# hrpan/tetris_mcts

Hardware: AMD Instinct MI355X
Metric: mcts_node_expansions_per_sec (higher is better)
Workload: dtype f32

## Files before the change

### include/tetris_mcts_hip.h

```cpp
#ifndef TETRIS_MCTS_HIP_H
#define TETRIS_MCTS_HIP_H
#include <stdint.h>
#ifdef __cplusplus
extern "C" {
#endif

#define TM_NACT 7
#define TM_GAME_DW 16
#define TM_OBS_DW 12
#define TM_REC_DW 32
#define TM_REC_PCHILD 28
#define TM_REC_OBS 29
#define TM_REC_SCORE 30
#define TM_REC_HDR 31
#define TM_KIDS_DW 8
#define TM_GS_DW 64
#define TM_LEAF_DW 32
#define TM_DIST_ROW 64
#define TM_GC_PART_DW 192
#define TM_VALUENET_PARAMS 478342
#define TM_VALUENET_SCRATCH 9728
#define TM_VALUENET_SCRATCH_MFMA 2064
#define TM_VALUENET_PREPARED 477184
#define TM_VALUENET_PREPARED_X3 27648
#define TM_VALUENET_FP32 0
#define TM_VALUENET_BF16X3 1
#define TM_DISTNET_PARAMS(atoms) (279232 + 129 * (atoms))
#define TM_DISTNET_PARAMS_50 285682
#define TM_DISTNET_PREPARED 278528
#define TM_DISTNET_PREPARED_X3 24576
#define TM_DISTNET_SCRATCH 2048

enum {
    TM_GS_ROOT = 0, TM_GS_EPISODE, TM_GS_NFREE_NODE, TM_GS_NFREE_OBS, TM_GS_TRACE_LEN, TM_GS_PENDING,
    TM_GS_ERR, TM_GS_N_EXPAND, TM_GS_N_SIMS, TM_GS_N_GC, TM_GS_RNG_POS, TM_GS_N_NQ_FALLBACK,
    TM_GS_LEAF, TM_GS_LEAF_END, TM_GS_K_EVAL, TM_GS_LEAF_SCORE,
    TM_GS_TRACE_SUM,
    TM_GS_N_EVAL,
    TM_GS_N_POOL_RESET,
    TM_GS_MAX_TRACE,
    TM_GS_CYC_BACK = 20, TM_GS_CYC_SELECT, TM_GS_CYC_EXPAND,
    TM_GS_CYC_TAIL,
    TM_GS_N_DROPPED = 25,
    TM_GS_LOW_NODE = 26, TM_GS_LOW_OBS,
    TM_GS_FIRST_MISS = 28,
    TM_GS_PREFIX_SUM,
    TM_GS_GC_PHASE = 32,
    TM_GS_GC_ARRIVE,
    TM_GS_GC_ACTIVE4,
    TM_GS_GC_RSV1,
    TM_GS_GC_WORK,
    TM_GS_GC_MARK_LAUNCHES,
    TM_GS_GC_SLICES,
    TM_GS_GC_RETRY,
    TM_GS_SIM_TARGET = 40, TM_GS_SIM_STARTED,
    TM_GS_CYC_VERIFY,
    TM_GS_N_WALK_MISS,
    TM_GS_POOL_FULL,
    TM_GS_GC_IN_MOVE,
    TM_GS_GC_REQ_AT,
    TM_GS_LEAF_OBS,
    TM_GS_N_EVAL_SKIP,
    TM_GS_N_EVAL_CACHED,
    TM_GS_GC_NGC,
    TM_GS_GC_BLOCKS,
    TM_GS_GC_ITERS,
    TM_GS_GC_MARK_CYC,
    TM_GS_GC_FLAGS
    , TM_GS_GC_MARK_PARTS = 58,
    TM_GS_GC_MARK_SHARED,
    TM_GS_GC_CYC_LOAD,
    TM_GS_GC_CYC_ROUNDS,
    TM_GS_GC_CYC_WAVES,
    TM_GS_GC_IDLE_TURNS
};
#define TM_GC_FLAG_WORDS 4
#define TM_ERR_POOL 1
#define TM_ERR_TRACE 2
#define TM_ERR_TABLE 4
#define TM_ERR_EVAL_LIST 8
#define TM_ERR_GC_GRID 16

#define TM_KIND_VALUESIM 0
#define TM_KIND_VALUESIM_LP 1
#define TM_KIND_CPPAGENT_LP 2
#define TM_KIND_CPPAGENT 3
#define TM_KIND_VANILLA 4
#define TM_KIND_VANILLA_C 5
#define TM_KIND_DIST 6

typedef struct tm_store {
    int32_t n_games;
    int32_t max_nodes;
    int32_t table_cap;
    int32_t max_trace;
    int32_t eval_slots;
    int32_t nq_size;
    int32_t app, scoring, randomizer;
    int32_t low;
    int32_t kind;
    int32_t min_visits_to_store;
    int32_t online;
    int32_t replay_cap;
    int32_t gc_slice_cycles;
    double gamma;
    uint32_t *node_rec;
    uint32_t *node_game;
    uint32_t *obs_stat;
    uint32_t *obs_key;
    uint64_t *node_tab;
    uint64_t *obs_tab;
    int32_t *free_node;
    int32_t *free_obs;
    int32_t *gs;
    uint32_t *rng;
    uint32_t *env_game;
    int32_t *env_line_stats;
    uint32_t *trace;
    int32_t *leaf;
    int32_t *eval_obs;
    float *eval_v;
    float *eval_var;
    const float *nq_table;
    uint8_t *gc_mark;
    int32_t *gc_queue;
    uint32_t *replay_obs;
    float *replay_stat;
    int32_t *replay_count;
    uint32_t *mt_state;
    uint32_t *node_child;
    int32_t *gc_part;
    float *node_dist;
    float *eval_dist;
    const double *nq_table_d;
    double dist_vmin, dist_vmax;
    int32_t dist_bins;
    int32_t gc_spec_nodes;
    int32_t *eval_list;
    int32_t *eval_cnt;
    float *obs_eval;
    int32_t eval_parity;
    int32_t eval_epoch;
    float *replay_dist;
    const int32_t *game_list;
    int32_t n_listed;
    int32_t gc_cost_units;
    int32_t gc_collectors;
} tm_store;
#define TM_EVAL_SEGS(n_games) ((n_games) < 64 ? (n_games) : 64)

int tm_pool_init(const tm_store *s, void *stream);
int tm_pool_reset(const tm_store *s, const uint8_t *mask, void *stream);
void tm_fill_norm_quantile(float *host_table, int n);
void tm_fill_norm_quantile_f64(double *host_table, int n);

int tm_env_init(const tm_store *s, const uint32_t *seeds, void *stream);
int tm_env_step(const tm_store *s, const int32_t *actions, void *stream);
int tm_env_reset(const tm_store *s, const uint8_t *mask, void *stream);
int tm_env_render(const tm_store *s, int8_t *out , void *stream);
int tm_env_info(const tm_store *s, int32_t *out , void *stream);

int tm_update_root(const tm_store *s, void *stream);
int tm_tree_new_node(const tm_store *s, const uint32_t *games, const uint8_t *mask, int32_t *out_idx, void *stream);
int tm_tree_expand(const tm_store *s, const uint32_t *games, const uint8_t *mask, int32_t *out_idx, void *stream);
int tm_tree_remove_nodes(const tm_store *s, const uint8_t *mask, void *stream);
int tm_move_begin(const tm_store *s, int sims, void *stream);
int tm_sims_remaining(const tm_store *s, int32_t *out , void *stream);
int tm_sims_owing(const tm_store *s, int32_t *out , int32_t *list, void *stream);
int tm_gc_step(const tm_store *s, void *stream);
#define TM_SIM_BACKUP 1
#define TM_SIM_FRONT 2
#define TM_SIM_GC_FULL 4
#define TM_SIM_EVAL_NEEDED 8
#define TM_SIM_GC_MEM_MARKS 16
int tm_sim_step(const tm_store *s, int flags, void *stream);
int tm_eval_render(const tm_store *s, int8_t *out , void *stream);

int tm_store_slice(const tm_store *s, int first, int n, tm_store *out);

typedef struct tm_search tm_search;
int tm_search_create(tm_search **out, const tm_store *s, int n_sub, int ev_every);
void tm_search_destroy(tm_search *h);
int tm_search_run(tm_search *h, int sims, const float *vn_params, const float *vn_prepared, float *vn_scratch,
                  void *stream);
int tm_search_stats(tm_search *h, double *out, int n, int reset);
int tm_search_set_epoch(tm_search *h, int epoch);
int tm_search_set_valuenet(tm_search *h, int backend);
int tm_root_stats(const tm_store *s, float *stats , int32_t *action , void *stream);
int tm_export_game(const tm_store *s, int game, int32_t *child , float *score, int32_t *n_to_o,
                   int32_t *visit, float *value, float *variance, uint8_t *end_obs, void *stream);

int tm_core_select_trace_obs(int n_trees, int n_nodes, const int32_t *roots, const int32_t *child,
                             const int32_t *visit, const float *value, const float *variance, const float *score,
                             const int32_t *n_to_o, int low, uint32_t *rng, const float *nq_table, int nq_size,
                             int32_t *trace , int32_t *trace_len, int max_trace, void *stream);
int tm_core_backup_trace_obs(int n_trees, int n_nodes, const int32_t *trace, const int32_t *trace_len, int max_trace,
                             int32_t *visit, float *value, float *variance, const int32_t *n_to_o, const float *score,
                             const double *_value, const double *_variance, double gamma, void *stream);
int tm_core_backup_trace_obs_lp(int n_trees, int n_nodes, const int32_t *trace, const int32_t *trace_len,
                                int max_trace, int32_t *visit, float *value, float *variance, const int32_t *n_to_o,
                                const float *score, const uint8_t *end, const int32_t *_child ,
                                const int32_t *_obs, const int32_t *k, const float *_value, const float *_variance,
                                double gamma, int mixture, int averaged, void *stream);
int tm_core_get_unique_child_obs(int n_trees, int n_nodes, const int32_t *index, const int32_t *child,
                                 const float *score, const int32_t *n_to_o, int32_t *c_nodes ,
                                 int32_t *c_obs, int32_t *count, void *stream);
int tm_core_get_all_childs(int n_trees, int n_nodes, const int32_t *roots, const int32_t *child,
                           uint8_t *mark , int32_t *queue , void *stream);

int tm_dist_transform(int n, int bins, const float *dist , double vmin, double vmax,
                      const double *shift , double scale, float *out , void *stream);
int tm_dist_mean_variance(int n, int bins, const float *dist, double vmin, double vmax, double *out ,
                          void *stream);

int tm_distpy_shift(int n, int bins, const float *dist , const double *x , double vmin, double vmax,
                    float *out , void *stream);
int tm_distpy_policy(int n_trees, int n_nodes, const int32_t *child_nodes, const int32_t *n_child, const float *node_stats,
                     const double *curr_reward , int32_t *out , void *stream);
int tm_distpy_backup(int n_trees, int n_nodes, int bins, const int32_t *trace, const int32_t *trace_len, int max_trace,
                     float *node_stats, float *node_dist, const double *r , const float *leaf_dist ,
                     double vmin, double vmax, float *scratch, void *stream);

int tm_yogi_step(float *p, const float *g, float *m, float *v, double *state, int n, double lr, double beta1, double beta2,
                 double eps, double weight_decay, void *stream);
int tm_valuenet_prepare(const float *params, float *prepared, void *stream);
int tm_valuenet_forward(const float *params, const float *prepared, const int8_t *states, int n, float *v, float *var,
                        float *scratch, void *stream);
int tm_valuenet_forward_requests(const float *params, const float *prepared, const tm_store *s, float *scratch,
                                 void *stream);
int tm_valuenet_forward_plain(const float *params, const int8_t *states, int n, float *v, float *var, float *scratch,
                              void *stream);
int tm_valuenet_prepare_x3(const float *params, float *prepared_x3, void *stream);
int tm_valuenet_forward_x3(const float *params, const float *prepared, const float *prepared_x3, const int8_t *states, int n,
                           float *v, float *var, float *scratch, void *stream);
int tm_valuenet_forward_requests_x3(const float *params, const float *prepared, const float *prepared_x3, const tm_store *s,
                                    float *scratch, void *stream);

int tm_distnet_prepare(const float *params, float *prepared, void *stream);
int tm_distnet_forward(const float *params, const float *prepared, const int8_t *states, int n, int atoms, float *dist,
                       int dist_stride, float *scratch, void *stream);
int tm_distnet_forward_requests(const float *params, const float *prepared, const tm_store *s, float *scratch, void *stream);
int tm_distnet_prepare_x3(const float *params, float *prepared_x3, void *stream);
int tm_distnet_forward_x3(const float *params, const float *prepared, const float *prepared_x3, const int8_t *states,
                          int n, int atoms, float *dist, int dist_stride, float *scratch, void *stream);
int tm_distnet_forward_requests_x3(const float *params, const float *prepared, const float *prepared_x3,
                                   const tm_store *s, float *scratch, void *stream);

const char *tm_version(void);
int tm_store_layout(int *out, int n);
#ifdef __cplusplus
}
#endif
#endif
```

### tetris_mcts_amd/csrc/valuenet.hip

```cpp
#include <hip/hip_runtime.h>
#include <stdint.h>
#include <stdlib.h>
#include <mutex>
#include "../../include/tetris_mcts_hip.h"

namespace tmcts_vn {

constexpr int A1 = 32 * 18 * 8, A2 = 32 * 16 * 6, A3 = 32 * 14 * 4, HID = 256;
constexpr int OFF_C1W = 0, OFF_C1B = 288, OFF_C2W = 320, OFF_C2B = 9536, OFF_C3W = 9568, OFF_C3B = 18784,
              OFF_F1W = 18816, OFF_F1B = 477568, OFF_FOW = 477824, OFF_FOB = 478336, OFF_UB = 478338, OFF_LB = 478340;

__device__ inline double tm_exp(double x) {
    if (x > 700.0) x = 700.0;
    if (x < -700.0) x = -700.0;
    const double inv_ln2 = 1.4426950408889634074, ln2_hi = 6.93147180369123816490e-01,
                 ln2_lo = 1.90821492927058770002e-10;
    double n = rint(x * inv_ln2);
    double r = fma(-n, ln2_hi, x);
    r = fma(-n, ln2_lo, r);
    double p = 1.0 / 6227020800.0;
    p = fma(p, r, 1.0 / 479001600.0);
    p = fma(p, r, 1.0 / 39916800.0);
    p = fma(p, r, 1.0 / 3628800.0);
    p = fma(p, r, 1.0 / 362880.0);
    p = fma(p, r, 1.0 / 40320.0);
    p = fma(p, r, 1.0 / 5040.0);
    p = fma(p, r, 1.0 / 720.0);
    p = fma(p, r, 1.0 / 120.0);
    p = fma(p, r, 1.0 / 24.0);
    p = fma(p, r, 1.0 / 6.0);
    p = fma(p, r, 0.5);
    p = fma(p, r, 1.0);
    p = fma(p, r, 1.0);
    long long bits = __double_as_longlong(p);
    bits += ((long long)n) << 52;
    return __longlong_as_double(bits);
}

template <int CIN, int H, int W>
__global__ void k_conv3x3_relu(const float* __restrict__ in, int in_stride, const int8_t* __restrict__ in8,
                               const float* __restrict__ wt, const float* __restrict__ bias, float* __restrict__ out,
                               int out_stride, int n) {
    constexpr int OH = H - 2, OW = W - 2, PER = 32 * OH * OW;
    int t = blockIdx.x * blockDim.x + threadIdx.x;
    if (t >= n * PER) return;
    int s = t / PER, e = t - s * PER;
    int co = e / (OH * OW), p = e - co * (OH * OW), y = p / OW, x = p - y * OW;
    float acc = bias[co];
    for (int ci = 0; ci < CIN; ++ci)
        for (int ky = 0; ky < 3; ++ky)
            for (int kx = 0; kx < 3; ++kx) {
                int ii = (ci * H + y + ky) * W + x + kx;
                float xv = in8 ? (float)in8[(size_t)s * 200 + ii] : in[(size_t)s * in_stride + ii];
                acc = fmaf(xv, wt[((co * CIN + ci) * 3 + ky) * 3 + kx], acc);
            }
    out[(size_t)s * out_stride + e] = acc > 0.0f ? acc : 0.0f;
}

__global__ void k_fc1_relu(const float* __restrict__ a3, int stride, const float* __restrict__ w,
                           const float* __restrict__ b, float* __restrict__ h, int hstride, int n) {
    int t = blockIdx.x * blockDim.x + threadIdx.x;
    if (t >= n * HID) return;
    int s = t / HID, j = t - s * HID;
    float acc = b[j];
    const float* x = a3 + (size_t)s * stride;
    const float* wr = w + (size_t)j * A3;
    for (int i = 0; i < A3; ++i) acc = fmaf(x[i], wr[i], acc);
    h[(size_t)s * hstride + j] = acc > 0.0f ? acc : 0.0f;
}

__global__ void k_fc_out(const float* __restrict__ h, int hstride, const float* __restrict__ P, float* __restrict__ v,
                         float* __restrict__ var, int n, const int32_t* __restrict__ eval_obs) {
    int t = blockIdx.x * blockDim.x + threadIdx.x;
    if (t >= n * 2) return;
    int s = t >> 1, j = t & 1;
    if (eval_obs && eval_obs[s] == 0) return;
    float acc = P[OFF_FOB + j];
    const float* x = h + (size_t)s * hstride;
    const float* wr = P + OFF_FOW + j * HID;
    for (int i = 0; i < HID; ++i) acc = fmaf(x[i], wr[i], acc);
    double e = tm_exp(-(double)acc);
    float sg = (float)(1.0 / (1.0 + e));
    float tt = sg * P[OFF_UB + j];
    float o = tt + P[OFF_LB + j];
    if (j == 0) v[s] = o; else var[s] = o;
}

}
namespace tmcts_vn {

typedef float f32x16 __attribute__((ext_vector_type(16)));
constexpr int SCHED_REGION_QUADS = 6;
constexpr int PREP_W2 = 0, PREP_W3 = 9216, PREP_W1 = 18432, PREP_TOTAL = 18432 + 458752;
constexpr int A1CS = 145;
constexpr int A2CS = 97;
constexpr int CONV_WG_PER_CU = 2;
constexpr int WAVE_LDS = 32 * A1CS + 200;

__global__ void k_vn_prepare(const float* __restrict__ P, float* __restrict__ prep) {
    int t = blockIdx.x * blockDim.x + threadIdx.x;
    if (t < 2 * 9216) {
        const float* W = P + (t < 9216 ? OFF_C2W : OFF_C3W);
        int e = t % 9216;
        int q = e / 256, l = (e / 4) % 64, r = e % 4;
        int s = 4 * q + r;
        int k = 2 * s + (l >> 5), row = l & 31;
        prep[t] = W[row * 288 + k];
    } else if (t < PREP_TOTAL) {
        int e = t - 18432;
        int ht = e / (112 * 256), e2 = e % (112 * 256);
        int q = e2 / 256, l = (e2 / 4) % 64, r = e2 % 4;
        int s = 4 * q + r;
        int k = 4 * s + (l >> 4), row = 16 * ht + (l & 15);
        prep[t] = P[OFF_F1W + (size_t)row * A3 + k];
    }
}

__device__ __forceinline__ void lds_fence() {
    __builtin_amdgcn_fence(__ATOMIC_RELEASE, "wavefront");
    __builtin_amdgcn_wave_barrier();
    __builtin_amdgcn_fence(__ATOMIC_ACQUIRE, "wavefront");
}

template <int TILES, int IN_CS>
__device__ __forceinline__ void conv_mfma(const float* __restrict__ in, const int (&boff)[TILES][9],
                                          const float4* __restrict__ W, f32x16 (&acc)[TILES]) {
    float4 wq[3];
    float bb[2][4][TILES];
    auto load_b = [&](int q, int buf) {
#pragma unroll
        for (int r = 0; r < 4; ++r) {
            const int s = 4 * q + r, cp = s / 9, j = s % 9;
#pragma unroll
            for (int t = 0; t < TILES; ++t) bb[buf][r][t] = in[boff[t][j] + cp * 2 * IN_CS];
        }
    };
    wq[0] = W[0];
    wq[1] = W[64];
    load_b(0, 0);
#pragma unroll
    for (int q = 0; q < 36; ++q) {
        if (q + 2 < 36) wq[(q + 2) % 3] = W[(q + 2) * 64];
        if (q + 1 < 36) load_b(q + 1, (q + 1) & 1);
        const float4 w4 = wq[q % 3];
#pragma unroll
        for (int r = 0; r < 4; ++r) {
            const float a = (r == 0) ? w4.x : (r == 1) ? w4.y : (r == 2) ? w4.z : w4.w;
#pragma unroll
            for (int t = 0; t < TILES; ++t)
                acc[t] = __builtin_amdgcn_mfma_f32_32x32x2f32(a, bb[q & 1][r][t], acc[t], 0, 0, 0);
        }
        __builtin_amdgcn_sched_group_barrier(0x020, 1, 0);
#pragma unroll
        for (int i = 0; i < 4 * TILES; ++i) {
            __builtin_amdgcn_sched_group_barrier(0x008, 1, 0);
            __builtin_amdgcn_sched_group_barrier(0x100, 1, 0);
        }
        if (q % SCHED_REGION_QUADS == SCHED_REGION_QUADS - 1) __builtin_amdgcn_sched_barrier(0);
    }
}

constexpr int CONV_WAVES_PER_SIMD = 2;
struct ReqList {
    const int2* list;
    const int32_t* cnt;
    int parity, segs, slots;
};
__device__ __forceinline__ int req_prefix(const ReqList& rq, int lane, int& total) {
    int incl = lane < rq.segs ? rq.cnt[lane * 2 + rq.parity] : 0;
#pragma unroll
    for (int d = 1; d < 64; d <<= 1) {
        const int t = __shfl_up(incl, d, 64);
        if (lane >= d) incl += t;
    }
    total = __shfl(incl, 63, 64);
    return incl;
}
__device__ __forceinline__ int req_at(const ReqList& rq, int incl, int p, int lane) {
    const int sg = __popcll(__ballot(lane < rq.segs && incl <= p));
    const int before = __shfl(incl, sg > 0 ? sg - 1 : 0, 64);
    const int d = p - (sg > 0 ? before : 0);
    return (sg + rq.segs * (d / rq.slots)) * rq.slots + d % rq.slots;
}
__device__ __forceinline__ uint32_t req_obs_word(const ReqList& rq, int incl, const uint32_t* __restrict__ obs_key, int max_nodes,
                                                 int n, int p, int lane) {
    if (p >= n) return 0u;
    const int2 e = rq.list[req_at(rq, incl, p, lane)];
    return lane < 12 ? obs_key[((size_t)(e.x / rq.slots) * max_nodes + e.y) * 12 + lane] : 0u;
}
__device__ __forceinline__ void render_obs(uint32_t kw, int lane, float* x0) {
    const uint32_t cells = __shfl((int)kw, 10, 64), endw = __shfl((int)kw, 11, 64);
#pragma unroll
    for (int it = 0; it < 4; ++it) {
        const int i = lane + 64 * it, ic = min(i, 199);
        int r = ic / 10, c = ic - 10 * r;
        uint32_t w2 = (uint32_t)__shfl((int)kw, r >> 1, 64);
        float v = (float)((w2 >> (16 * (r & 1) + c)) & 1u);
        bool pc = ((cells & 0xFF) == (uint32_t)ic) | (((cells >> 8) & 0xFF) == (uint32_t)ic) |
                  (((cells >> 16) & 0xFF) == (uint32_t)ic) | ((cells >> 24) == (uint32_t)ic);
        if (!(endw & 0xFFu) && pc) v = -1.0f;
        if (i < 200) x0[i] = v;
    }
}
#include "valuenet_conv.inc"

typedef float f32x4 __attribute__((ext_vector_type(4)));
typedef float f32x4v __attribute__((ext_vector_type(4)));
#ifdef TM_FC1_TIMELINE
#define FC1_STAMP(i) do { if (threadIdx.x == 0 && s0 + (int)blockIdx.y < n) reinterpret_cast<int*>(hout)[(size_t)(s0 + blockIdx.y) * hstride + HID + 1 + (i)] = (int)__builtin_amdgcn_s_memrealtime(); } while (0)
#else
#define FC1_STAMP(i) do { } while (0)
#endif
template <int RT, int NY, int KC, int WRING, int PF>
__global__ __launch_bounds__(512) void k_vn_fc1(const float* __restrict__ P, const float* __restrict__ prep,
                                                const float* __restrict__ a3, int a3stride, int n,
                                                float* __restrict__ hout, int hstride,
                                                ReqList rq, int32_t* __restrict__ cnt, int cnt_stride,
                                                float* __restrict__ v_out, float* __restrict__ var_out) {
    constexpr int ROWS = 16 * RT, PITCH = KC + 4, HS_PITCH = HID + 4;
    constexpr int UNITS = HID / NY, HT = UNITS / 16, SG = 8 / HT, NST = RT / SG;
    static_assert(HT * SG == 8 && NST * SG == RT && NST >= 1 && ROWS <= 64, "eight waves = hidden tiles x groups of state tiles; one lane per row");
    constexpr int BT = ROWS * PITCH > (ROWS * HS_PITCH + 1) / 2 ? ROWS * PITCH : (ROWS * HS_PITCH + 1) / 2;
    __shared__ __attribute__((aligned(16))) float bt[2][BT];
    __shared__ int row_slot[ROWS];
    __shared__ int last_flag;
    const int w = threadIdx.x >> 6, lane = threadIdx.x & 63, kk = lane >> 4, l15 = lane & 15;
    const int s0 = blockIdx.x * ROWS;
    int my_slot = 0;
    FC1_STAMP(0);
    if (rq.list) {
        const int incl = req_prefix(rq, lane, n);
        if (s0 >= n) return;
        if (w == 0) {
            const int p = min(s0 + (lane & (ROWS - 1)), n - 1);
            int sg = 0;
            for (int k = 0; k < rq.segs; ++k) sg += __builtin_amdgcn_readlane(incl, k) <= p ? 1 : 0;
            const int before = __shfl(incl, sg > 0 ? sg - 1 : 0, 64);
            const int d = p - (sg > 0 ? before : 0);
            my_slot = rq.list[(sg + rq.segs * (d / rq.slots)) * rq.slots + d % rq.slots].x;
        }
    }
    const int ht = blockIdx.y * HT + (w % HT);
    const int st0 = (w / HT) * NST;
    const float4* W = reinterpret_cast<const float4*>(prep + PREP_W1) + (size_t)ht * 112 * 64 + lane;
    f32x4 acc[NST];
#pragma unroll
    for (int t = 0; t < NST; ++t)
#pragma unroll
        for (int r = 0; r < 4; ++r) acc[t][r] = P[OFF_F1B + 16 * ht + kk * 4 + r];
    constexpr int NCH = A3 / KC;
    constexpr int GRP = 16 / NST, QPG = GRP / 4, NGRP = KC / 4 / GRP;
    static_assert(A3 % KC == 0 && NCH >= 2 && (KC / 4) % GRP == 0, "chunking");
    float4 wring[WRING][QPG];
    auto wload = [&](int G) {
#pragma unroll
        for (int q = 0; q < QPG; ++q) wring[G % WRING][q] = W[((size_t)G * QPG + q) * 64];
    };
#pragma unroll
    for (int G0 = 0; G0 < WRING - 1; ++G0) wload(G0);
    constexpr int TPR = KC / 4, RPP = 512 / TPR, NPASS = ROWS / RPP;
    const int row0 = threadIdx.x / TPR, c4 = (threadIdx.x % TPR) * 4;
    float4 st[PF][NPASS];
    auto gload = [&](int chunk) {
#pragma unroll
        for (int i = 0; i < NPASS; ++i) {
            const int sa = s0 + row0 + RPP * i;
            st[chunk % PF][i] = (sa < n) ? *reinterpret_cast<const float4*>(a3 + (size_t)sa * a3stride + chunk * KC + c4)
                                         : make_float4(0, 0, 0, 0);
        }
    };
    auto lstore = [&](int chunk) {
#pragma unroll
        for (int i = 0; i < NPASS; ++i)
            *reinterpret_cast<float4*>(&bt[chunk & 1][(row0 + RPP * i) * PITCH + c4]) = st[chunk % PF][i];
    };
    static_assert(PF >= 2 && PF <= A3 / KC, "chunks in flight");
#pragma unroll
    for (int c = 0; c < PF; ++c) gload(c);
    FC1_STAMP(1);
    lstore(0);
    __syncthreads();
    FC1_STAMP(2);
#pragma unroll
    for (int c = 0; c < NCH; ++c) {
        if (c + PF < NCH) gload(c + PF);
        const float* b0 = &bt[c & 1][(16 * st0 + l15) * PITCH + kk];
        float bb[2][NST][GRP];
        auto load_b = [&](int grp, int buf) {
#pragma unroll
            for (int t = 0; t < NST; ++t)
#pragma unroll
                for (int i = 0; i < GRP; ++i) bb[buf][t][i] = b0[16 * t * PITCH + 4 * (GRP * grp + i)];
        };
        load_b(0, 0);
#pragma unroll
        for (int gq = 0; gq < NGRP; ++gq) {
            const int G = c * NGRP + gq;
            if (G + WRING - 1 < NCH * NGRP) wload(G + WRING - 1);
            if (gq + 1 < NGRP) load_b(gq + 1, (gq + 1) & 1);
#pragma unroll
            for (int i = 0; i < GRP; ++i) {
                const float4 w4 = wring[G % WRING][i / 4];
                const int r = i & 3;
                const float a = (r == 0) ? w4.x : (r == 1) ? w4.y : (r == 2) ? w4.z : w4.w;
#pragma unroll
                for (int t = 0; t < NST; ++t)
                    acc[t] = __builtin_amdgcn_mfma_f32_16x16x4f32(a, bb[gq & 1][t][i], acc[t], 0, 0, 0);
            }
#pragma unroll
            for (int i = 0; i < NST * GRP / 2; ++i) {
                __builtin_amdgcn_sched_group_barrier(0x008, 2, 0);
                __builtin_amdgcn_sched_group_barrier(0x100, 1, 0);
            }
            __builtin_amdgcn_sched_barrier(0);
        }
        if (c + 1 < NCH) lstore(c + 1);
        __syncthreads();
        if (c == NCH - 1) FC1_STAMP(3);
    }
    const int i0 = 16 * ht + kk * 4;
    float* hs = &bt[0][0];
    static_assert(ROWS * HS_PITCH <= 2 * BT, "hidden tile fits the staging buffers");
#pragma unroll
    for (int t = 0; t < NST; ++t) {
        f32x4v o0;
#pragma unroll
        for (int r = 0; r < 4; ++r) o0[r] = acc[t][r] > 0.f ? acc[t][r] : 0.f;
        const int row = 16 * (st0 + t) + l15;
        if (s0 + row < n) {
            float* dst = hout + (size_t)(s0 + row) * hstride + i0;
            asm volatile("global_store_dwordx4 %0, %1, off sc1" :: "v"(dst), "v"(o0) : "memory");
        }
        *reinterpret_cast<f32x4v*>(&hs[row * HS_PITCH + i0]) = o0;
    }
    if (rq.list && w == 0 && lane < ROWS) row_slot[lane] = my_slot;
    asm volatile("s_waitcnt vmcnt(0)" ::: "memory");
    __syncthreads();
    FC1_STAMP(4);
    if (threadIdx.x == 0) {
        const int old = __hip_atomic_fetch_add(&cnt[(size_t)blockIdx.x * cnt_stride], 1, __ATOMIC_RELAXED, __HIP_MEMORY_SCOPE_AGENT);
        last_flag = old;
        if (old == NY - 1) __hip_atomic_store(&cnt[(size_t)blockIdx.x * cnt_stride], 0, __ATOMIC_RELAXED, __HIP_MEMORY_SCOPE_AGENT);
    }
    __syncthreads();
    FC1_STAMP(5);
    if (last_flag != NY - 1) return;
    {
        constexpr int OQ = (HID - UNITS) / 4, CNT = ROWS * OQ / 512;
        static_assert(ROWS * OQ % 512 == 0, "whole passes");
        f32x4v wv[CNT];
#pragma unroll
        for (int i = 0; i < CNT; ++i) {
            const int e = i * 512 + threadIdx.x, row = e / OQ, c = (e % OQ) * 4;
            const int col = c < (int)blockIdx.y * UNITS ? c : c + UNITS;
            const float* src = hout + (size_t)(s0 + (s0 + row < n ? row : 0)) * hstride + col;
            asm volatile("global_load_dwordx4 %0, %1, off sc1" : "=v"(wv[i]) : "v"(src) : "memory");
        }
        asm volatile("s_waitcnt vmcnt(0)" ::: "memory");
#pragma unroll
        for (int i = 0; i < CNT; ++i) {
            const int e = i * 512 + threadIdx.x, row = e / OQ, c = (e % OQ) * 4;
            const int col = c < (int)blockIdx.y * UNITS ? c : c + UNITS;
            f32x4v t = wv[i];
            asm volatile("" : "+v"(t));
            if (s0 + row < n) *reinterpret_cast<f32x4v*>(&hs[row * HS_PITCH + col]) = t;
        }
    }
    __syncthreads();
    FC1_STAMP(6);
    if (threadIdx.x < 2 * ROWS) {
        const int j = threadIdx.x >> 1, o = threadIdx.x & 1;
        int sidx = s0 + j;
        const bool live = sidx < n;
        if (rq.list) sidx = row_slot[j];
        if (live) {
            float a = P[OFF_FOB + o];
            const float* x = &hs[j * HS_PITCH];
            const float* wr = P + OFF_FOW + o * HID;
            if ((reinterpret_cast<uintptr_t>(wr) & 15) == 0) {
                const float4* x4 = reinterpret_cast<const float4*>(x);
                const float4* w4 = reinterpret_cast<const float4*>(wr);
#pragma unroll 8
                for (int i = 0; i < HID / 4; ++i) {
                    const float4 xv = x4[i], wv = w4[i];
                    a = fmaf(xv.x, wv.x, a); a = fmaf(xv.y, wv.y, a); a = fmaf(xv.z, wv.z, a); a = fmaf(xv.w, wv.w, a);
                }
            } else {
#pragma unroll 8
                for (int i = 0; i < HID; ++i) a = fmaf(x[i], wr[i], a);
            }
            const double e = tm_exp(-(double)a);
            const float sg = (float)(1.0 / (1.0 + e));
            const float tt = sg * P[OFF_UB + o];
            const float res = tt + P[OFF_LB + o];
            if (o == 0) v_out[sidx] = res; else var_out[sidx] = res;
        }
    }
    FC1_STAMP(7);
}

#include "valuenet_x3.inc"

}

using namespace tmcts_vn;

extern "C" {

int tm_valuenet_prepare(const float* P, float* prepared, void* stream_) {
    hipLaunchKernelGGL(k_vn_prepare, dim3((PREP_TOTAL + 255) / 256), dim3(256), 0, (hipStream_t)stream_, P, prepared);
    return (int)hipGetLastError();
}

int tm_valuenet_forward_plain(const float* P, const int8_t* states, int n, float* v, float* var, float* scratch,
                              void* stream_) {
    hipStream_t stream = (hipStream_t)stream_;
    if (n <= 0) return 0;
    constexpr int SS = TM_VALUENET_SCRATCH;
    float* a1 = scratch;
    const int T = 256;
    hipLaunchKernelGGL((k_conv3x3_relu<1, 20, 10>), dim3((n * A1 + T - 1) / T), dim3(T), 0, stream, (const float*)nullptr,
                       0, states, P + OFF_C1W, P + OFF_C1B, a1, SS, n);
    hipLaunchKernelGGL((k_conv3x3_relu<32, 18, 8>), dim3((n * A2 + T - 1) / T), dim3(T), 0, stream, a1, SS,
                       (const int8_t*)nullptr, P + OFF_C2W, P + OFF_C2B, a1 + A1, SS, n);
    hipLaunchKernelGGL((k_conv3x3_relu<32, 16, 6>), dim3((n * A3 + T - 1) / T), dim3(T), 0, stream, a1 + A1, SS,
                       (const int8_t*)nullptr, P + OFF_C3W, P + OFF_C3B, a1 + A1 + A2, SS, n);
    hipLaunchKernelGGL(k_fc1_relu, dim3((n * HID + T - 1) / T), dim3(T), 0, stream, a1 + A1 + A2, SS, P + OFF_F1W,
                       P + OFF_F1B, a1 + A1 + A2 + A3, SS, n);
    hipLaunchKernelGGL(k_fc_out, dim3((n * 2 + T - 1) / T), dim3(T), 0, stream, a1 + A1 + A2 + A3, SS, P, v, var, n,
                       (const int32_t*)nullptr);
    return (int)hipGetLastError();
}

static int vn_forward_impl(const float* P, const float* prepared, const __bf16* planes, const int8_t* states,
                           const uint32_t* obs_key, const ReqList& rq, int max_nodes, int n, float* v, float* var,
                           float* scratch, hipStream_t stream) {
    if (n <= 0) return 0;
    constexpr int SS = TM_VALUENET_SCRATCH_MFMA;
    static_assert(SS >= A3 + HID + 1 && SS % 4 == 0, "scratch row");
    if (planes) {
        const int lds = 4 * X3_WAVE_BYTES;
        static std::once_flag x3_once;
        static int x3_err = 0;
        std::call_once(x3_once, [&] {
            x3_err = (int)hipFuncSetAttribute(reinterpret_cast<const void*>(k_vn_conv_x3),
                                              hipFuncAttributeMaxDynamicSharedMemorySize, lds);
        });
        if (x3_err) return x3_err;
        const int blocks = (n + 3) / 4 < 256 ? (n + 3) / 4 : 256;
        hipLaunchKernelGGL(k_vn_conv_x3, dim3(blocks), dim3(256), lds, stream, P, planes, states, obs_key, rq,
                           max_nodes, n, scratch, SS, reinterpret_cast<int32_t*>(scratch + A3 + HID), 32 * SS);
    } else {
        const int lds = 4 * WAVE_LDS * (int)sizeof(float);
        static std::once_flag attr_once;
        static int attr_err = 0;
        std::call_once(attr_once, [&] {
            attr_err = (int)hipFuncSetAttribute(reinterpret_cast<const void*>(k_vn_conv),
                                                hipFuncAttributeMaxDynamicSharedMemorySize, lds);
        });
        if (attr_err) return attr_err;
        int blocks = (n + 3) / 4;
        if (blocks > 256 * CONV_WG_PER_CU) blocks = 256 * CONV_WG_PER_CU;
        hipLaunchKernelGGL(k_vn_conv, dim3(blocks), dim3(256), lds, stream, P, prepared, states, obs_key, rq,
                           max_nodes, n, scratch, SS, reinterpret_cast<int32_t*>(scratch + A3 + HID), 32 * SS);
    }
    if (n >= 8192)
        hipLaunchKernelGGL((k_vn_fc1<4, 4, 128, 3, 2>), dim3((n + 63) / 64, 4), dim3(512), 0, stream, P, prepared, scratch, SS, n,
                           scratch + A3, SS, rq, reinterpret_cast<int32_t*>(scratch + A3 + HID), 64 * SS, v, var);
    else
        hipLaunchKernelGGL((k_vn_fc1<2, 4, 256, 6, 2>), dim3((n + 31) / 32, 4), dim3(512), 0, stream, P, prepared, scratch, SS, n,
                           scratch + A3, SS, rq, reinterpret_cast<int32_t*>(scratch + A3 + HID), 32 * SS, v, var);
    return (int)hipGetLastError();
}

int tm_valuenet_forward(const float* P, const float* prepared, const int8_t* states, int n, float* v, float* var,
                        float* scratch, void* stream_) {
    return vn_forward_impl(P, prepared, nullptr, states, nullptr, ReqList{nullptr, nullptr, 0, 0, 1}, 0, n, v, var, scratch,
                           (hipStream_t)stream_);
}

int tm_valuenet_forward_requests(const float* P, const float* prepared, const tm_store* s, float* scratch, void* stream_) {
    const ReqList rq{reinterpret_cast<const int2*>(s->eval_list), s->eval_cnt, s->eval_parity, TM_EVAL_SEGS(s->n_games), s->eval_slots};
    return vn_forward_impl(P, prepared, nullptr, nullptr, s->obs_key, rq, s->max_nodes,
                           s->n_games * s->eval_slots, s->eval_v, s->eval_var, scratch, (hipStream_t)stream_);
}

int tm_valuenet_prepare_x3(const float* P, float* prepared_x3, void* stream_) {
    if (!prepared_x3) return (int)hipErrorInvalidValue;
    hipLaunchKernelGGL(k_vn_prepare_x3, dim3((2 * 18 * 64 * 8 + 255) / 256), dim3(256), 0, (hipStream_t)stream_, P,
                       reinterpret_cast<__bf16*>(prepared_x3));
    return (int)hipGetLastError();
}

int tm_valuenet_forward_x3(const float* P, const float* prepared, const float* prepared_x3, const int8_t* states, int n, float* v,
                           float* var, float* scratch, void* stream_) {
    if (!prepared_x3) return (int)hipErrorInvalidValue;
    return vn_forward_impl(P, prepared, reinterpret_cast<const __bf16*>(prepared_x3), states, nullptr,
                           ReqList{nullptr, nullptr, 0, 0, 1}, 0, n, v, var, scratch, (hipStream_t)stream_);
}

int tm_valuenet_forward_requests_x3(const float* P, const float* prepared, const float* prepared_x3, const tm_store* s,
                                    float* scratch, void* stream_) {
    if (!prepared_x3) return (int)hipErrorInvalidValue;
    const ReqList rq{reinterpret_cast<const int2*>(s->eval_list), s->eval_cnt, s->eval_parity, TM_EVAL_SEGS(s->n_games), s->eval_slots};
    return vn_forward_impl(P, prepared, reinterpret_cast<const __bf16*>(prepared_x3), nullptr, s->obs_key, rq, s->max_nodes,
                           s->n_games * s->eval_slots, s->eval_v, s->eval_var, scratch, (hipStream_t)stream_);
}

}
```

Baseline: 20.32 million.

## Make valuenet fc1 a persistent grid dealing tile/part items across CUs

Replaces the 2D grid of fc1 blocks (tiles x hidden parts) with a persistent grid sized to resident workgroups per CU, where each block loops over (tile, part) items dealt in an XCD-aware order. The request prefix is computed once per block instead of per tile, and the output-layer weights are staged into LDS during the last chunk instead of read from global memory in the epilogue. Adds a waves-per-EU attribute and a non-inlined sigmoid to reduce register pressure. This targets launch overhead and tail imbalance, at the cost of extra per-item syncs and loop overhead.

```diff
diff --git a/include/tetris_mcts_hip.h b/include/tetris_mcts_hip.h
--- a/include/tetris_mcts_hip.h
+++ b/include/tetris_mcts_hip.h
@@ -230,6 +230,7 @@
                                  void *stream);
 int tm_valuenet_forward_plain(const float *params, const int8_t *states, int n, float *v, float *var, float *scratch,
                               void *stream);
+int tm_fc1_deal(int requests, int rows, int parts, int grid, int b, int32_t *items, int cap);
 int tm_valuenet_prepare_x3(const float *params, float *prepared_x3, void *stream);
 int tm_valuenet_forward_x3(const float *params, const float *prepared, const float *prepared_x3, const int8_t *states, int n,
                            float *v, float *var, float *scratch, void *stream);
diff --git a/tetris_mcts_amd/csrc/valuenet.hip b/tetris_mcts_amd/csrc/valuenet.hip
--- a/tetris_mcts_amd/csrc/valuenet.hip
+++ b/tetris_mcts_amd/csrc/valuenet.hip
@@ -206,13 +206,29 @@
 
 typedef float f32x4 __attribute__((ext_vector_type(4)));
 typedef float f32x4v __attribute__((ext_vector_type(4)));
+constexpr int FC1_XCDS = 8;
+struct Fc1Item { int tile, part; };
+__host__ __device__ constexpr int fc1_item_count(int requests, int rows, int parts) {
+    return requests > 0 ? (requests + rows - 1) / rows * parts : 0;
+}
+__host__ __device__ constexpr int fc1_item_index(int b, int grid, int k) { return b + k * grid; }
+__host__ __device__ constexpr Fc1Item fc1_item(int index, int requests, int rows, int parts) {
+    const int tiles = (requests + rows - 1) / rows, t8 = tiles / FC1_XCDS * FC1_XCDS, bulk = t8 * parts;
+    if (index < bulk) return Fc1Item{index % t8, index / t8};
+    const int rest = tiles - t8, j = index - bulk;
+    return Fc1Item{t8 + j % rest, j / rest};
+}
 #ifdef TM_FC1_TIMELINE
-#define FC1_STAMP(i) do { if (threadIdx.x == 0 && s0 + (int)blockIdx.y < n) reinterpret_cast<int*>(hout)[(size_t)(s0 + blockIdx.y) * hstride + HID + 1 + (i)] = (int)__builtin_amdgcn_s_memrealtime(); } while (0)
+#define FC1_STAMP(i) do { if (tid == 0 && s0 + part < n) reinterpret_cast<int*>(hout)[(size_t)(s0 + part) * hstride + HID + 1 + (i)] = (int)__builtin_amdgcn_s_memrealtime(); } while (0)
 #else
 #define FC1_STAMP(i) do { } while (0)
 #endif
+__device__ __noinline__ float fc1_sigmoid(float a) {
+    const double e = tm_exp(-(double)a);
+    return (float)(1.0 / (1.0 + e));
+}
 template <int RT, int NY, int KC, int WRING, int PF>
-__global__ __launch_bounds__(512) void k_vn_fc1(const float* __restrict__ P, const float* __restrict__ prep,
+__global__ __launch_bounds__(512) __attribute__((amdgpu_waves_per_eu(RT == 4 ? 4 : 2))) void k_vn_fc1(const float* __restrict__ P, const float* __restrict__ prep,
                                                 const float* __restrict__ a3, int a3stride, int n,
                                                 float* __restrict__ hout, int hstride,
                                                 ReqList rq, int32_t* __restrict__ cnt, int cnt_stride,
@@ -224,13 +240,25 @@
     __shared__ __attribute__((aligned(16))) float bt[2][BT];
     __shared__ int row_slot[ROWS];
     __shared__ int last_flag;
-    const int w = threadIdx.x >> 6, lane = threadIdx.x & 63, kk = lane >> 4, l15 = lane & 15;
-    const int s0 = blockIdx.x * ROWS;
+    constexpr int WO = 2 * HID + 6;
+    static_assert(OFF_FOB == OFF_FOW + 2 * HID && OFF_UB == OFF_FOB + 2 && OFF_LB == OFF_UB + 2, "the output layer's parameters are consecutive");
+    __shared__ __attribute__((aligned(16))) float wo[(WO + 3) / 4 * 4];
+    const int lane = threadIdx.x & 63;
+    int incl = 0;
+    if (rq.list) {
+        incl = req_prefix(rq, lane, n);
+        n = __builtin_amdgcn_readfirstlane(n);
+    }
+    const int n_items = fc1_item_count(n, ROWS, NY);
+    for (int item = fc1_item_index(blockIdx.x, gridDim.x, 0), kth = 0; item < n_items; item = fc1_item_index(blockIdx.x, gridDim.x, ++kth)) {
+    int tid = threadIdx.x;
+    asm volatile("" : "+v"(tid));
+    const int w = tid >> 6, lane = tid & 63, kk = lane >> 4, l15 = lane & 15;
+    const Fc1Item it = fc1_item(item, n, ROWS, NY);
+    const int tile = it.tile, part = it.part, s0 = tile * ROWS;
     int my_slot = 0;
     FC1_STAMP(0);
     if (rq.list) {
-        const int incl = req_prefix(rq, lane, n);
-        if (s0 >= n) return;
         if (w == 0) {
             const int p = min(s0 + (lane & (ROWS - 1)), n - 1);
             int sg = 0;
@@ -240,7 +268,7 @@
             my_slot = rq.list[(sg + rq.segs * (d / rq.slots)) * rq.slots + d % rq.slots].x;
         }
     }
-    const int ht = blockIdx.y * HT + (w % HT);
+    const int ht = part * HT + (w % HT);
     const int st0 = (w / HT) * NST;
     const float4* W = reinterpret_cast<const float4*>(prep + PREP_W1) + (size_t)ht * 112 * 64 + lane;
     f32x4 acc[NST];
@@ -259,7 +287,7 @@
 #pragma unroll
     for (int G0 = 0; G0 < WRING - 1; ++G0) wload(G0);
     constexpr int TPR = KC / 4, RPP = 512 / TPR, NPASS = ROWS / RPP;
-    const int row0 = threadIdx.x / TPR, c4 = (threadIdx.x % TPR) * 4;
+    const int row0 = tid / TPR, c4 = (tid % TPR) * 4;
     float4 st[PF][NPASS];
     auto gload = [&](int chunk) {
 #pragma unroll
@@ -275,6 +303,7 @@
             *reinterpret_cast<float4*>(&bt[chunk & 1][(row0 + RPP * i) * PITCH + c4]) = st[chunk % PF][i];
     };
     static_assert(PF >= 2 && PF <= A3 / KC, "chunks in flight");
+    float wo_r[4] = {0.f, 0.f, 0.f, 0.f};
 #pragma unroll
     for (int c = 0; c < PF; ++c) gload(c);
     FC1_STAMP(1);
@@ -284,6 +313,11 @@
 #pragma unroll
     for (int c = 0; c < NCH; ++c) {
         if (c + PF < NCH) gload(c + PF);
+        if (c == NCH - 1 && tid < (WO + 3) / 4) {
+#pragma unroll
+            for (int r = 0; r < 4; ++r)
+                if (4 * tid + r < WO) wo_r[r] = P[OFF_FOW + 4 * tid + r];
+        }
         const float* b0 = &bt[c & 1][(16 * st0 + l15) * PITCH + kk];
         float bb[2][NST][GRP];
         auto load_b = [&](int grp, int buf) {
@@ -334,33 +368,34 @@
         *reinterpret_cast<f32x4v*>(&hs[row * HS_PITCH + i0]) = o0;
     }
     if (rq.list && w == 0 && lane < ROWS) row_slot[lane] = my_slot;
+    if (tid < (WO + 3) / 4) *reinterpret_cast<float4*>(&wo[4 * tid]) = make_float4(wo_r[0], wo_r[1], wo_r[2], wo_r[3]);
     asm volatile("s_waitcnt vmcnt(0)" ::: "memory");
     __syncthreads();
     FC1_STAMP(4);
-    if (threadIdx.x == 0) {
-        const int old = __hip_atomic_fetch_add(&cnt[(size_t)blockIdx.x * cnt_stride], 1, __ATOMIC_RELAXED, __HIP_MEMORY_SCOPE_AGENT);
+    if (tid == 0) {
+        const int old = __hip_atomic_fetch_add(&cnt[(size_t)tile * cnt_stride], 1, __ATOMIC_RELAXED, __HIP_MEMORY_SCOPE_AGENT);
         last_flag = old;
-        if (old == NY - 1) __hip_atomic_store(&cnt[(size_t)blockIdx.x * cnt_stride], 0, __ATOMIC_RELAXED, __HIP_MEMORY_SCOPE_AGENT);
+        if (old == NY - 1) __hip_atomic_store(&cnt[(size_t)tile * cnt_stride], 0, __ATOMIC_RELAXED, __HIP_MEMORY_SCOPE_AGENT);
     }
     __syncthreads();
     FC1_STAMP(5);
-    if (last_flag != NY - 1) return;
+    if (last_flag == NY - 1) {
     {
         constexpr int OQ = (HID - UNITS) / 4, CNT = ROWS * OQ / 512;
         static_assert(ROWS * OQ % 512 == 0, "whole passes");
         f32x4v wv[CNT];
 #pragma unroll
         for (int i = 0; i < CNT; ++i) {
-            const int e = i * 512 + threadIdx.x, row = e / OQ, c = (e % OQ) * 4;
-            const int col = c < (int)blockIdx.y * UNITS ? c : c + UNITS;
+            const int e = i * 512 + tid, row = e / OQ, c = (e % OQ) * 4;
+            const int col = c < part * UNITS ? c : c + UNITS;
             const float* src = hout + (size_t)(s0 + (s0 + row < n ? row : 0)) * hstride + col;
             asm volatile("global_load_dwordx4 %0, %1, off sc1" : "=v"(wv[i]) : "v"(src) : "memory");
         }
         asm volatile("s_waitcnt vmcnt(0)" ::: "memory");
 #pragma unroll
         for (int i = 0; i < CNT; ++i) {
-            const int e = i * 512 + threadIdx.x, row = e / OQ, c = (e % OQ) * 4;
-            const int col = c < (int)blockIdx.y * UNITS ? c : c + UNITS;
+            const int e = i * 512 + tid, row = e / OQ, c = (e % OQ) * 4;
+            const int col = c < part * UNITS ? c : c + UNITS;
             f32x4v t = wv[i];
             asm volatile("" : "+v"(t));
             if (s0 + row < n) *reinterpret_cast<f32x4v*>(&hs[row * HS_PITCH + col]) = t;
@@ -368,35 +403,30 @@
     }
     __syncthreads();
     FC1_STAMP(6);
-    if (threadIdx.x < 2 * ROWS) {
-        const int j = threadIdx.x >> 1, o = threadIdx.x & 1;
+    if (tid < 2 * ROWS) {
+        const int j = tid >> 1, o = tid & 1;
         int sidx = s0 + j;
         const bool live = sidx < n;
         if (rq.list) sidx = row_slot[j];
         if (live) {
-            float a = P[OFF_FOB + o];
-            const float* x = &hs[j * HS_PITCH];
-            const float* wr = P + OFF_FOW + o * HID;
-            if ((reinterpret_cast<uintptr_t>(wr) & 15) == 0) {
-                const float4* x4 = reinterpret_cast<const float4*>(x);
-                const float4* w4 = reinterpret_cast<const float4*>(wr);
+            float a = wo[2 * HID + o];
+            const float4* x4 = reinterpret_cast<const float4*>(&hs[j * HS_PITCH]);
+            const float4* w4 = reinterpret_cast<const float4*>(&wo[o * HID]);
 #pragma unroll 8
-                for (int i = 0; i < HID / 4; ++i) {
-                    const float4 xv = x4[i], wv = w4[i];
-                    a = fmaf(xv.x, wv.x, a); a = fmaf(xv.y, wv.y, a); a = fmaf(xv.z, wv.z, a); a = fmaf(xv.w, wv.w, a);
-                }
-            } else {
-#pragma unroll 8
-                for (int i = 0; i < HID; ++i) a = fmaf(x[i], wr[i], a);
+            for (int i = 0; i < HID / 4; ++i) {
+                const float4 xv = x4[i], wv = w4[i];
+                a = fmaf(xv.x, wv.x, a); a = fmaf(xv.y, wv.y, a); a = fmaf(xv.z, wv.z, a); a = fmaf(xv.w, wv.w, a);
             }
-            const double e = tm_exp(-(double)a);
-            const float sg = (float)(1.0 / (1.0 + e));
-            const float tt = sg * P[OFF_UB + o];
-            const float res = tt + P[OFF_LB + o];
+            const float sg = fc1_sigmoid(a);
+            const float tt = sg * wo[2 * HID + 2 + o];
+            const float res = tt + wo[2 * HID + 4 + o];
             if (o == 0) v_out[sidx] = res; else var_out[sidx] = res;
         }
     }
     FC1_STAMP(7);
+    }
+    if (fc1_item_index(blockIdx.x, gridDim.x, kth + 1) < n_items) __syncthreads();
+    }
 }
 
 #include "valuenet_x3.inc"
@@ -404,6 +434,35 @@
 }
 
 using namespace tmcts_vn;
+
+static int vn_compute_units() {
+    static std::once_flag once;
+    static int cus = 0;
+    std::call_once(once, [&] {
+        int dev = 0;
+        if (hipGetDevice(&dev) != hipSuccess || hipDeviceGetAttribute(&cus, hipDeviceAttributeMultiprocessorCount, dev) != hipSuccess) cus = 0;
+    });
+    return cus;
+}
+
+template <int RT, int NY, int KC, int WRING, int PF, int WG_PER_CU>
+static int vn_fc1_launch_shape(const float* P, const float* prepared, const ReqList& rq, int n, float* v, float* var,
+                               float* scratch, hipStream_t stream) {
+    constexpr int SS = TM_VALUENET_SCRATCH_MFMA, ROWS = 16 * RT;
+    const int cus = vn_compute_units();
+    if (cus <= 0) return (int)hipErrorInvalidDevice;
+    const int items = fc1_item_count(n, ROWS, NY), resident = cus * WG_PER_CU;
+    hipLaunchKernelGGL((k_vn_fc1<RT, NY, KC, WRING, PF>), dim3(items < resident ? items : resident), dim3(512), 0, stream, P,
+                       prepared, scratch, SS, n, scratch + A3, SS, rq, reinterpret_cast<int32_t*>(scratch + A3 + HID), ROWS * SS,
+                       v, var);
+    return (int)hipGetLastError();
+}
+static int vn_fc1_launch(const float* P, const float* prepared, const ReqList& rq, int n, float* v, float* var, float* scratch,
+                         hipStream_t stream) {
+    if (n >= 8192)
+        return vn_fc1_launch_shape<4, 4, 128, 3, 2, 2>(P, prepared, rq, n, v, var, scratch, stream);
+    return vn_fc1_launch_shape<2, 4, 256, 6, 2, 1>(P, prepared, rq, n, v, var, scratch, stream);
+}
 
 extern "C" {
 
@@ -464,13 +523,7 @@
         hipLaunchKernelGGL(k_vn_conv, dim3(blocks), dim3(256), lds, stream, P, prepared, states, obs_key, rq,
                            max_nodes, n, scratch, SS, reinterpret_cast<int32_t*>(scratch + A3 + HID), 32 * SS);
     }
-    if (n >= 8192)
-        hipLaunchKernelGGL((k_vn_fc1<4, 4, 128, 3, 2>), dim3((n + 63) / 64, 4), dim3(512), 0, stream, P, prepared, scratch, SS, n,
-                           scratch + A3, SS, rq, reinterpret_cast<int32_t*>(scratch + A3 + HID), 64 * SS, v, var);
-    else
-        hipLaunchKernelGGL((k_vn_fc1<2, 4, 256, 6, 2>), dim3((n + 31) / 32, 4), dim3(512), 0, stream, P, prepared, scratch, SS, n,
-                           scratch + A3, SS, rq, reinterpret_cast<int32_t*>(scratch + A3 + HID), 32 * SS, v, var);
-    return (int)hipGetLastError();
+    return vn_fc1_launch(P, prepared, rq, n, v, var, scratch, stream);
 }
 
 int tm_valuenet_forward(const float* P, const float* prepared, const int8_t* states, int n, float* v, float* var,
@@ -483,6 +536,17 @@
     const ReqList rq{reinterpret_cast<const int2*>(s->eval_list), s->eval_cnt, s->eval_parity, TM_EVAL_SEGS(s->n_games), s->eval_slots};
     return vn_forward_impl(P, prepared, nullptr, nullptr, s->obs_key, rq, s->max_nodes,
                            s->n_games * s->eval_slots, s->eval_v, s->eval_var, scratch, (hipStream_t)stream_);
+}
+
+int tm_fc1_deal(int requests, int rows, int parts, int grid, int b, int32_t* items, int cap) {
+    if (requests < 0 || rows <= 0 || parts <= 0 || grid <= 0 || b < 0 || b >= grid) return -1;
+    const int n_items = fc1_item_count(requests, rows, parts);
+    int k = 0;
+    for (int i = fc1_item_index(b, grid, 0); i < n_items; i = fc1_item_index(b, grid, ++k)) {
+        const Fc1Item it = fc1_item(i, requests, rows, parts);
+        if (items && k < cap) { items[2 * k] = it.tile; items[2 * k + 1] = it.part; }
+    }
+    return k;
 }
 
 int tm_valuenet_prepare_x3(const float* P, float* prepared_x3, void* stream_) {
```

Result: faster. 20.70 million, median of 6 (+1.9%).
